# deevinandu/Distributed-Multi-Agent-SLAM-Swarm-Robotics-System

Hardware: NVIDIA B200
Metric: beam_cell_updates_per_sec (higher is better)
Workload: dtype f64+u32

## Files before the change

### distributed-multi-agent-slam-swarm-robotics-system_b200/csrc/beam_expand.cuh

```cuda
#pragma once
#include "sincos_dd.cuh"

namespace occ {

struct Geom {
    double ox, oy, res;
    double inv_res;
    int size_x, size_y;
    int win_x0, win_y0, win_w, win_h;
};

struct Beam {
    int x0, y0, x1, y1;
    int hit;
    int valid;
    int slow;
};

#define OCC_MAX_DIST_M 1.20
#define OCC_MIN_DIST_M 0.05
#define OCC_CELL_LIMIT 1073741824.0

OCC_HD float load_f32_unaligned(const uint8_t* p) {
    uint32_t v = (uint32_t)p[0] | ((uint32_t)p[1] << 8) | ((uint32_t)p[2] << 16) | ((uint32_t)p[3] << 24);
#if defined(__CUDA_ARCH__)
    return __uint_as_float(v);
#else
    float f;
    __builtin_memcpy(&f, &v, 4);
    return f;
#endif
}

OCC_HD double cell_quotient(double w, double o, double res) { return OCC_DDIV(OCC_DADD(w, -o), res); }

OCC_HD bool quotient_in_range(double q) { return fabs(q) < OCC_CELL_LIMIT; }

OCC_HD int trunc_cell(double q) {
#if defined(__CUDA_ARCH__)
    return __double2int_rz(q);
#else
    return (int)q;
#endif
}

OCC_HD double screening_tolerance(double r, double o, double yaw, double inv_res) {
    return OCC_DMUL(OCC_DMUL(fabs(r) + fabs(o) + fabs(yaw) + 11.0, inv_res), 0x1p-47);
}

OCC_HD bool near_cell_boundary(double q, double tol) { return !(fabs(q - rint(q)) > tol); }

struct LibSinCos {
    OCC_HD_MEMBER void operator()(double a, double* s, double* c) const {
#if defined(__CUDA_ARCH__)
        sincos(a, s, c);
#else
        *s = sin(a);
        *c = cos(a);
#endif
    }
};

OCC_HD double sensor_angle(int s) {
    const double h = 0x1.921fb54442d18p+0;
    return s == 0 ? 0.0 : (s == 1 ? h : (s == 2 ? 0x1.921fb54442d18p+1 : -h));
}

template <class FastSinCos>
OCC_HD void expand_beam(const Geom& g, double rx, double ry, double ryaw, int x0, int y0, bool origin_ok,
                        int sensor, float dist_f32, double sn, double cs, double tolx, double toly,
                        const FastSinCos& fsc, Beam* b) {
    double dist = (double)dist_f32;
    bool hit = (OCC_MIN_DIST_M < dist) && (dist <= OCC_MAX_DIST_M);
    double range = hit ? dist : OCC_MAX_DIST_M;
    double qx = OCC_DMUL(OCC_DADD(OCC_DADD(rx, OCC_DMUL(range, cs)), -g.ox), g.inv_res);
    double qy = OCC_DMUL(OCC_DADD(OCC_DADD(ry, OCC_DMUL(range, sn)), -g.oy), g.inv_res);
    int slow = 0;
    if (near_cell_boundary(qx, tolx) || near_cell_boundary(qy, toly)) {
        double ang = OCC_DADD(ryaw, sensor_angle(sensor));
        double s2, c2;
        if (!sincos_dd(ang, &s2, &c2)) fsc(ang, &s2, &c2);
        qx = cell_quotient(OCC_DADD(rx, OCC_DMUL(range, c2)), g.ox, g.res);
        qy = cell_quotient(OCC_DADD(ry, OCC_DMUL(range, s2)), g.oy, g.res);
        slow = 1;
    }
    b->hit = hit ? 1 : 0;
    b->slow = slow;
    b->x0 = x0;
    b->y0 = y0;
    bool ok = origin_ok && quotient_in_range(qx) && quotient_in_range(qy);
    b->valid = ok ? 1 : 0;
    b->x1 = ok ? trunc_cell(qx) : 0;
    b->y1 = ok ? trunc_cell(qy) : 0;
}

enum { PKT_OK = 0, PKT_DROPPED = 1, PKT_BAD_POSE = 2 };

OCC_HD int decode_packet(const uint8_t* p, long long k, const int32_t* agent_idx, const double* drift,
                         const double* agent_off, int n_agents,
                         double* rx, double* ry, double* ryaw, float dist[4], int* agent_out = nullptr) {
    if (!(p[0] == 'Q' && p[1] == 'S' && p[2] == 'R' && p[3] == 'L')) return PKT_DROPPED;
    long long agent = agent_idx ? (long long)agent_idx[k] : (long long)p[4];
    if (agent < 1 || agent > n_agents) return PKT_DROPPED;
// ... 107 lines not shown
```

### distributed-multi-agent-slam-swarm-robotics-system_b200/csrc/occgrid_tiled.cu

```cuda
#include "common.cuh"

namespace occ {

constexpr int kTT = 256;
constexpr int kChunkPk = 2048;
constexpr int kChunkMin = 256;
constexpr int kItemsPerCta = 3;
constexpr int kMaxWindowBytes = 100 * 1024;

struct TilePlanHeader {
    unsigned int n_items, n_active, total_records, work_counter, resolve_counter, overflow;
    unsigned int active_count;
    unsigned int pad;
};

__device__ __forceinline__ int home_tile(const Geom& g, const TileGeom& tg, double rx, double ry) {
    const double qx = cell_quotient(rx, g.ox, g.res), qy = cell_quotient(ry, g.oy, g.res);
    if (!quotient_in_range(qx) || !quotient_in_range(qy)) return -1;
    const int px = trunc_cell(qx) - g.win_x0 + tg.pad, py = trunc_cell(qy) - g.win_y0 + tg.pad;
    if (px < tg.pad - tg.reach || py < tg.pad - tg.reach || px >= tg.pad + g.win_w + tg.reach ||
        py >= tg.pad + g.win_h + tg.reach)
        return -1;
    return (py >> kTileShift) * tg.tiles_x + (px >> kTileShift);
}

constexpr int kPkPerCta = 2048;
constexpr int kSub = kPkPerCta / kTT;
constexpr int kHash = 4096;
constexpr unsigned int kEmpty = 0xffffffffu;
static_assert(kHash >= 2 * kPkPerCta, "hash table must stay at most half full");

__device__ __forceinline__ int hash_insert(unsigned int* keys, unsigned int tile) {
    unsigned int h = (tile * 2654435761u) >> 20;
    for (;;) {
        const unsigned int old = atomicCAS(&keys[h], kEmpty, tile);
        if (old == kEmpty || old == tile) return (int)h;
        h = (h + 1) & (kHash - 1);
    }
}

constexpr int kHashPerThread = kHash / kTT;

__device__ __forceinline__ void flush_tile_counts(const unsigned int* s_keys, const unsigned int* s_vals,
                                                  unsigned int* __restrict__ tile_count, unsigned int* __restrict__ active,
                                                  TilePlanHeader* __restrict__ hdr) {
    unsigned int key[kHashPerThread], old[kHashPerThread];
#pragma unroll
    for (int j = 0; j < kHashPerThread; ++j) {
        const int i = j * kTT + threadIdx.x;
        key[j] = s_keys[i];
        old[j] = 1u;
        if (key[j] != kEmpty) old[j] = atomicAdd(&tile_count[key[j]], s_vals[i]);
    }
#pragma unroll
    for (int j = 0; j < kHashPerThread; ++j)
        if (key[j] != kEmpty && old[j] == 0u) active[atomicAdd(&hdr->active_count, 1u)] = key[j];
}

__device__ __forceinline__ void reserve_tile_ranges(const unsigned int* s_keys, unsigned int* s_vals,
                                                    const unsigned int* __restrict__ tile_offset, unsigned int* __restrict__ tile_cursor) {
    unsigned int key[kHashPerThread], base[kHashPerThread], off[kHashPerThread];
#pragma unroll
    for (int j = 0; j < kHashPerThread; ++j) {
        const int i = j * kTT + threadIdx.x;
        key[j] = s_keys[i];
        base[j] = off[j] = 0u;
        if (key[j] != kEmpty) { off[j] = tile_offset[key[j]]; base[j] = atomicAdd(&tile_cursor[key[j]], s_vals[i]); }
    }
#pragma unroll
    for (int j = 0; j < kHashPerThread; ++j)
        if (key[j] != kEmpty) s_vals[j * kTT + threadIdx.x] = off[j] + base[j];
}

constexpr size_t kBinSmem = (size_t)kTT * kMaxRecStride + 2 * kHash * sizeof(unsigned int) + kPkPerCta * sizeof(unsigned short);
constexpr unsigned int kNoSlot = 0xffffu;

template <bool kMaps = false>
__global__ void __launch_bounds__(kTT)
k_home_bin(Geom g, TileGeom tg, const uint8_t* __restrict__ pkts, long long n, int stride,
           const int32_t* __restrict__ agent_idx, const double* __restrict__ drift,
           const double* __restrict__ agent_off, int n_agents,
           unsigned int* __restrict__ tile_count, PoseRec* __restrict__ recs, unsigned int* __restrict__ local_bins, uint2* __restrict__ runs,
           unsigned int* __restrict__ seg_count, unsigned int* __restrict__ active, TilePlanHeader* __restrict__ hdr,
           uint64_t* counters) {
    extern __shared__ __align__(16) uint8_t s_bin[];
    uint8_t* const s_rec = s_bin;
    unsigned int* const s_keys = reinterpret_cast<unsigned int*>(s_bin + kTT * kMaxRecStride);
    unsigned int* const s_vals = s_keys + kHash;
    unsigned short* const s_slot = reinterpret_cast<unsigned short*>(s_vals + kHash);
    __shared__ unsigned int s_wsum[kTT / 32];
    for (int i = threadIdx.x; i < kHash; i += kTT) { s_keys[i] = kEmpty; s_vals[i] = 0u; }
    unsigned long long c[OCCGRID_C_HITS + 1] = {};
    const long long cta_first = (long long)blockIdx.x * kPkPerCta;
    constexpr int kVec = (kTT * kMaxRecStride / 16 + kTT - 1) / kTT;
    uint4 pre[kVec];
    auto prefetch = [&](int sub) {
        const long long first = cta_first + (long long)sub * kTT;
        const long long left = n - first;
        const size_t bytes = left <= 0 ? 0 : (size_t)min((long long)kTT, left) * stride;
        const uint4* s4 = reinterpret_cast<const uint4*>(pkts + (size_t)first * stride);
#pragma unroll
        for (int j = 0; j < kVec; ++j) {
            const size_t i = (size_t)j * kTT + threadIdx.x;
            pre[j] = (i * 16 + 16 <= bytes) ? __ldg(s4 + i) : make_uint4(0u, 0u, 0u, 0u);
        }
    };
    const bool vec_ok = (reinterpret_cast<uintptr_t>(pkts) & 15) == 0 && ((kTT * stride) & 15) == 0;
    if (vec_ok) prefetch(0);
    for (int sub = 0; sub < kSub; ++sub) {
        const long long first = cta_first + (long long)sub * kTT;
        if (first >= n) break;
        const int count = (int)min((long long)kTT, n - first);
        __syncthreads();
        if (vec_ok) {
            const size_t bytes = (size_t)count * stride;
            uint4* d4 = reinterpret_cast<uint4*>(s_rec);
#pragma unroll
            for (int j = 0; j < kVec; ++j) {
                const size_t i = (size_t)j * kTT + threadIdx.x;
                if (i * 16 + 16 <= bytes) d4[i] = pre[j];
            }
            for (size_t i = (bytes / 16) * 16 + threadIdx.x; i < bytes; i += kTT) s_rec[i] = __ldg(pkts + (size_t)first * stride + i);
            if (sub + 1 < kSub) prefetch(sub + 1);
        } else {
            stage_records(pkts + (size_t)first * stride, (size_t)count * stride, s_rec);
        }
        __syncthreads();
        if ((int)threadIdx.x < count) {
            const long long k = first + threadIdx.x;
            double rx, ry, ryaw;
            float dist[4];
            c[OCCGRID_C_PACKETS] += 1;
            unsigned int slot = kNoSlot;
            int agent = 1;
            const int st = decode_packet(s_rec + threadIdx.x * stride, k, agent_idx, drift, agent_off, n_agents, &rx, &ry, &ryaw, dist,
                                         kMaps ? &agent : nullptr);
            if (st == PKT_DROPPED) c[OCCGRID_C_DROPPED] += 1;
            else if (st == PKT_BAD_POSE) c[OCCGRID_C_BAD_POSE] += 1;
            else {
                c[OCCGRID_C_ACCEPTED] += 1;
                c[OCCGRID_C_BEAMS] += 4;
#pragma unroll
                for (int s = 0; s < 4; ++s) {
                    const double d = (double)dist[s];
                    c[OCCGRID_C_HITS] += (OCC_MIN_DIST_M < d && d <= OCC_MAX_DIST_M) ? 1 : 0;
                }
                int tile = home_tile(g, tg, rx, ry);
                if (kMaps && tile >= 0) tile += (agent - 1) * tg.n_tiles;
                if (tile >= 0) {
                    slot = (unsigned int)hash_insert(s_keys, (unsigned int)tile);
                    atomicAdd(&s_vals[slot], 1u);
                    PoseRec r;
                    r.rx = rx; r.ry = ry; r.yaw = (float)ryaw;
                    r.d[0] = dist[0]; r.d[1] = dist[1]; r.d[2] = dist[2]; r.d[3] = dist[3];
                    r.k = (unsigned int)k;
                    r.tile = tile; r.pad = 0;
                    recs[k] = r;
                }
            }
            s_slot[sub * kTT + threadIdx.x] = (unsigned short)slot;
        }
    }
    __syncthreads();
    unsigned int key[kHashPerThread], rank[kHashPerThread];
#pragma unroll
    for (int j = 0; j < kHashPerThread; ++j) {
        const int i = j * kTT + threadIdx.x;
        key[j] = s_keys[i];
        rank[j] = 0u;
        if (key[j] != kEmpty) rank[j] = atomicAdd(&tile_count[key[j]], s_vals[i]);
    }
    const int lane = threadIdx.x & 31, warp = threadIdx.x >> 5;
    unsigned int mine = 0u;
#pragma unroll
    for (int j = 0; j < kHashPerThread; ++j) mine += key[j] != kEmpty ? s_vals[j * kTT + threadIdx.x] + 0x10000u : 0u;
    unsigned int inc = mine;
#pragma unroll
    for (int o = 1; o < 32; o <<= 1) { const unsigned int u = __shfl_up_sync(0xffffffffu, inc, o); if (lane >= o) inc += u; }
    if (lane == 31) s_wsum[warp] = inc;
    __syncthreads();
    unsigned int pos = inc - mine, n_local = 0u;
#pragma unroll
    for (int w = 0; w < kTT / 32; ++w) {
        pos += w < warp ? s_wsum[w] : 0u;
        n_local += s_wsum[w];
    }
    n_local &= 0xffffu;
    if (threadIdx.x == 0) seg_count[blockIdx.x] = n_local;
    const size_t seg0 = (size_t)blockIdx.x * kPkPerCta;
#pragma unroll
    for (int j = 0; j < kHashPerThread; ++j) {
        if (key[j] == kEmpty) continue;
        const int i = j * kTT + threadIdx.x;
        const unsigned int run = pos >> 16, begin = pos & 0xffffu;
        runs[seg0 + run] = make_uint2(key[j], rank[j] - begin);
        pos += s_vals[i] + 0x10000u;
        s_keys[i] = run;
        s_vals[i] = begin;
        if (rank[j] == 0u) active[atomicAdd(&hdr->active_count, 1u)] = key[j];
    }
    __syncthreads();
    unsigned int* const s_local = reinterpret_cast<unsigned int*>(s_rec);
    const int n_seg = (int)min((long long)kPkPerCta, n - (long long)seg0);
    for (int j = threadIdx.x; j < n_seg; j += kTT) {
        const unsigned int slot = s_slot[j];
        if (slot != kNoSlot) s_local[atomicAdd(&s_vals[slot], 1u)] = (s_keys[slot] << 16) | (unsigned int)j;
    }
    __syncthreads();
    for (unsigned int j = threadIdx.x; j < n_local; j += kTT) local_bins[seg0 + j] = s_local[j];
    __syncthreads();
    block_add_counters(c, reinterpret_cast<unsigned long long*>(s_rec), counters);
}

__global__ void __launch_bounds__(kTT)
k_place_runs(const unsigned int* __restrict__ local_bins, const uint2* __restrict__ runs, const unsigned int* __restrict__ seg_count,
             const unsigned int* __restrict__ tile_offset, const TilePlanHeader* __restrict__ hdr, unsigned int* __restrict__ bins) {
    if (hdr->overflow) return;
    const size_t seg0 = (size_t)blockIdx.x * kPkPerCta;
    const int n_local = (int)seg_count[blockIdx.x];
    unsigned int e[kSub], off[kSub];
    uint2 d[kSub];
#pragma unroll
    for (int sub = 0; sub < kSub; ++sub) {
        const int j = sub * kTT + threadIdx.x;
        e[sub] = j < n_local ? local_bins[seg0 + j] : kEmpty;
    }
#pragma unroll
    for (int sub = 0; sub < kSub; ++sub) d[sub] = e[sub] != kEmpty ? runs[seg0 + (e[sub] >> 16)] : make_uint2(0u, 0u);
#pragma unroll
    for (int sub = 0; sub < kSub; ++sub) off[sub] = e[sub] != kEmpty ? tile_offset[d[sub].x] : 0u;
#pragma unroll
    for (int sub = 0; sub < kSub; ++sub)
        if (e[sub] != kEmpty) bins[off[sub] + d[sub].y + (unsigned int)(sub * kTT + threadIdx.x)] = (unsigned int)(seg0 + (e[sub] & 0xffffu));
}

__device__ __forceinline__ int chunk_valid(const SegInfo& seg, long long chunk, long long* addr0) {
    const long long a0 = chunk * kSegChunk;
    *addr0 = a0;
    const unsigned int sg = (unsigned int)(a0 / seg.seg_cap);
    const unsigned int j0 = (unsigned int)(a0 - (long long)sg * seg.seg_cap);
    unsigned int cnt = seg.d_counts ? seg.d_counts[sg] : seg.host_count;
    if (cnt > seg.seg_cap) cnt = seg.seg_cap;
    return cnt > j0 ? (int)min((unsigned int)kSegChunk, cnt - j0) : 0;
}

__global__ void __launch_bounds__(kTT)
k_home_count_poses(Geom g, TileGeom tg, const PoseRec* __restrict__ recs, const int* __restrict__ in_tiles, SegInfo seg, long long n_chunks,
                   int tiles_in_records,
                   unsigned int* __restrict__ tile_count, int* __restrict__ tile_ids,
                   unsigned int* __restrict__ active, TilePlanHeader* __restrict__ hdr, uint64_t* counters) {
    __shared__ unsigned int s_keys[kHash];
    __shared__ unsigned int s_vals[kHash];
    __shared__ unsigned long long s_acc[(OCCGRID_C_HITS + 1) * 32];
    unsigned long long c[OCCGRID_C_HITS + 1] = {};
    for (long long chunk = blockIdx.x; chunk < n_chunks; chunk += gridDim.x) {
        long long addr0;
        const int valid = chunk_valid(seg, chunk, &addr0);
        if (valid == 0) continue;
        for (int i = threadIdx.x; i < kHash; i += kTT) { s_keys[i] = kEmpty; s_vals[i] = 0u; }
        __syncthreads();
        if (tiles_in_records) {
            int tl[kSub];
#pragma unroll
            for (int sub = 0; sub < kSub; ++sub) {
// ... 268 lines not shown
    else      asm volatile("red.shared.max.u32 [%0], %1;" ::"r"(addr), "r"(v) : "memory");
}

template <bool kAdd>
__device__ __forceinline__ void walk_beam_masked(unsigned int win, int pitch, int x, int y, int ddx, int ddy,
                                                 unsigned int v_free, bool hit, bool skip_first, const unsigned int* s_mask) {
    const int dx = abs(ddx), dy = abs(ddy);
    const bool xmajor = dx >= dy;
    const int dmaj = xmajor ? dx : dy, dmin = xmajor ? dy : dx;
    const int sx4 = ddx > 0 ? 4 : -4;
    const int sy4 = (ddy > 0 ? pitch : -pitch) * 4;
    const int step_maj = xmajor ? sx4 : sy4, step_min = xmajor ? sy4 : sx4;
    unsigned int mask = s_mask[dmaj * (dmaj + 1) / 2 + dmin];
    unsigned int a = win + (unsigned int)(y * pitch + x) * 4u;
    const unsigned int a_end = a + (unsigned int)((ddy * pitch + ddx) * 4);
    int rem = dmaj;
    if (rem > 0) {
        if (!skip_first) smem_red<kAdd>(a, v_free);
        a += step_maj + ((mask & 1u) ? step_min : 0);
        mask >>= 1;
        --rem;
    }
    while (rem >= 8) {
#pragma unroll
        for (int j = 0; j < 8; ++j) {
            smem_red<kAdd>(a, v_free);
            a += step_maj + ((mask & (1u << j)) ? step_min : 0);
        }
        mask >>= 8;
        rem -= 8;
    }
    if (rem >= 4) {
#pragma unroll
        for (int j = 0; j < 4; ++j) {
            smem_red<kAdd>(a, v_free);
            a += step_maj + ((mask & (1u << j)) ? step_min : 0);
        }
        mask >>= 4;
        rem -= 4;
    }
    for (; rem > 0; --rem) {
        smem_red<kAdd>(a, v_free);
        a += step_maj + ((mask & 1u) ? step_min : 0);
        mask >>= 1;
    }
    if (hit && !(dmaj == 0 && skip_first && !kAdd)) smem_red<kAdd>(a_end, kAdd ? 0x10000u : (v_free | 1u));
}

struct RouteSmem {
    unsigned int cnt[kMaxBands];
    unsigned int off[kMaxBands + 1];
    unsigned int base[kMaxBands];
};

__device__ __forceinline__ unsigned int lds_u32_at(const unsigned int* __restrict__ words, unsigned int byte_off) {
    const unsigned int w = byte_off >> 2, sh = (byte_off & 3u) * 8u;
    return __funnelshift_r(words[w], words[w + 1], sh);
}

__device__ __forceinline__ int decode_packet_smem(const unsigned int* __restrict__ words, unsigned int byte_off, long long k,
                                                  const int32_t* agent_idx, const double* drift, const double* agent_off,
                                                  int n_agents, double* rx, double* ry, float* yaw, float dist[4]) {
    if (lds_u32_at(words, byte_off) != 0x4c525351u) return PKT_DROPPED;
    const unsigned int b4 = lds_u32_at(words, byte_off + 4);
    const long long agent = agent_idx ? (long long)agent_idx[k] : (long long)(b4 & 0xffu);
    if (agent < 1 || agent > n_agents) return PKT_DROPPED;
    const unsigned int b8 = lds_u32_at(words, byte_off + 8), b12 = lds_u32_at(words, byte_off + 12),
                       b16 = lds_u32_at(words, byte_off + 16);
    double x = (double)__uint_as_float(__funnelshift_r(b4, b8, 8));
    double y = (double)__uint_as_float(__funnelshift_r(b8, b12, 8));
    const float fyaw = __uint_as_float(__funnelshift_r(b12, b16, 8));
    x = OCC_DADD(x, agent_off[2 * agent + 0]);
    y = OCC_DADD(y, agent_off[2 * agent + 1]);
    if (drift) {
        const double2 dv = *reinterpret_cast<const double2*>(drift + 2 * k);
        x = OCC_DADD(x, dv.x);
        y = OCC_DADD(y, dv.y);
    }
    if (!(isfinite(x) && isfinite(y) && isfinite(fyaw))) return PKT_BAD_POSE;
    *rx = x; *ry = y; *yaw = fyaw;
    const unsigned int c24 = lds_u32_at(words, byte_off + 24), c28 = lds_u32_at(words, byte_off + 28),
                       c32 = lds_u32_at(words, byte_off + 32), c36 = lds_u32_at(words, byte_off + 36),
                       c40 = lds_u32_at(words, byte_off + 40);
    dist[0] = __uint_as_float(__funnelshift_r(c24, c28, 8));
    dist[1] = __uint_as_float(__funnelshift_r(c28, c32, 8));
    dist[2] = __uint_as_float(__funnelshift_r(c32, c36, 8));
    dist[3] = __uint_as_float(__funnelshift_r(c36, c40, 8));
    return PKT_OK;
}

__device__ __forceinline__ bool robot_cell(double r, double o, double res, double inv_res, int* cell) {
    double q = OCC_DMUL(OCC_DADD(r, -o), inv_res);
    const double tol = OCC_DMUL(OCC_DMUL(fabs(r) + fabs(o) + 11.0, inv_res), 0x1p-47);
    if (near_cell_boundary(q, tol)) q = cell_quotient(r, o, res);
    if (!quotient_in_range(q)) return false;
    *cell = trunc_cell(q);
    return true;
}

struct RouteStats { unsigned int a, b; };

constexpr int kRouteSubs = kRouteSubsPerItem;
constexpr int kRoutePerThread = kRouteItemPk / kTT;
static_assert(kRouteItemPk % kTT == 0 && kRoutePerThread >= 1 && kRoutePerThread <= 4, "route sub-batch = 1..4 packets per thread");

struct RoutePk {
    double rx, ry;
    float yaw, d[4];
    int band0, nb, tile0, tile1;
    unsigned int rank0, rank1;
};

__device__ __forceinline__ void route_decode(const RouteJob& J, const unsigned int* s_buf, int slot, long long k, RoutePk& P,
                                             RouteStats& st_acc) {
    P.band0 = -1; P.nb = 0; P.tile0 = P.tile1 = -1; P.rank0 = P.rank1 = 0u;
    const int st = decode_packet_smem(s_buf, (unsigned int)slot * (unsigned int)J.stride, k, J.agent_idx, J.drift, J.agent_off,
                                      J.n_agents, &P.rx, &P.ry, &P.yaw, P.d);
    st_acc.a += 1u + (st == PKT_OK ? 0x10000u : 0u);
    st_acc.b += st == PKT_DROPPED ? 1u : 0u;
    if (st != PKT_OK) return;
    unsigned int hits = 0;
#pragma unroll
    for (int s2 = 0; s2 < 4; ++s2) {
        const double dd = (double)P.d[s2];
        hits += (OCC_MIN_DIST_M < dd && dd <= OCC_MAX_DIST_M) ? 1u : 0u;
    }
    st_acc.b += hits << 16;
    int gx, gy;
    if (!(robot_cell(P.rx, J.ox, J.res, J.inv_res, &gx) && robot_cell(P.ry, J.oy, J.res, J.inv_res, &gy))) return;
    const int reach = J.reach;
    if (gx < -reach || gx >= J.size_x + reach) return;
    const int tcol = (gx + J.pad) >> kTileShift;
    for (int b = 0; b < J.n_bands; ++b) {
        if (gy - reach < J.band_y0[b + 1]) {
            const int py = gy - J.band_y0[b];
            if (py >= -reach) {
                P.band0 = b; P.nb = 1;
                P.tile0 = ((py + J.pad) >> kTileShift) * J.tiles_x + tcol;
                if (b + 1 < J.n_bands && gy + reach >= J.band_y0[b + 1]) {
                    P.nb = 2;
                    P.tile1 = ((gy - J.band_y0[b + 1] + J.pad) >> kTileShift) * J.tiles_x + tcol;
                }
            }
            break;
        }
    }
}

__device__ __forceinline__ void route_rank(RouteSmem& S, RoutePk& P, int lane, unsigned int lt) {
    const unsigned int p0 = __match_any_sync(0xffffffffu, P.band0);
    if (P.band0 >= 0) {
// ... 208 lines not shown
        if (threadIdx.x == 0) next_pos = atomicAdd(&hdr->work_counter, 1u);
        __syncthreads();
        {
            const int lx_lo = max(0, g.win_x0 - wx0), lx_hi = min(side, g.win_x0 + g.win_w - wx0);
            const int ly_lo = max(0, g.win_y0 - wy0), ly_hi = min(side, g.win_y0 + g.win_h - wy0);
            const int lane = threadIdx.x & 31, warp = threadIdx.x >> 5;
            for (int ly = warp; ly < side; ly += kTT / 32) {
                unsigned int* row = s_win + ly * pitch;
                const bool row_in = ly >= ly_lo && ly < ly_hi;
                unsigned int* out = plane + (size_t)(wy0 + ly - g.win_y0) * g.win_w + (wx0 - g.win_x0);
                for (int lx = lane; lx < side; lx += 32) {
                    const unsigned int v = row[lx];
                    if (!v) continue;
                    if (!kRoute) row[lx] = 0u;
                    if (!(row_in && lx >= lx_lo && lx < lx_hi)) continue;
                    if (kCounts)
                        atomicAdd(reinterpret_cast<unsigned long long*>(plane) + ((size_t)(wy0 + ly - g.win_y0) * g.win_w + (wx0 - g.win_x0) + lx),
                                  ((unsigned long long)(v >> 16) << 32) | (unsigned long long)(v & 0xffffu));
                    else
                        atomicMax(out + lx, v);
                }
            }
        }
        if (threadIdx.x == 0) s_next[turn ^ 1] = next_pos;
        __syncthreads();
    }
    if (kRoute && job.counters) {
        __syncthreads();
        const unsigned long long pk = rs.a & 0xffffu, acc = rs.a >> 16, drp = rs.b & 0xffffu, hits = rs.b >> 16;
        const unsigned long long rc[6] = {pk, acc, drp, pk - acc - drp, 4ull * acc, hits};
        block_add_counters(rc, s_acc, job.counters);
    }
    if (counters) {
        __syncthreads();
        const int lane = threadIdx.x & 31, warp = threadIdx.x >> 5;
#pragma unroll
        for (int i = 0; i < 3; ++i) {
            unsigned long long x = c[i];
#pragma unroll
            for (int o = 16; o > 0; o >>= 1) x += __shfl_xor_sync(0xffffffffu, x, o);
            if (lane == 0) s_acc[i * 32 + warp] = x;
        }
        __syncthreads();
        if (threadIdx.x < 3) {
            unsigned long long t = 0;
            for (int w = 0; w < kTT / 32; ++w) t += s_acc[threadIdx.x * 32 + w];
            const int slot = threadIdx.x == 0 ? OCCGRID_C_UPDATES : (threadIdx.x == 1 ? OCCGRID_C_SLOWPATH : OCCGRID_C_OWNED_UPDATES);
            if (t) atomicAdd(reinterpret_cast<unsigned long long*>(counters) + slot, t);
        }
    }
}

constexpr int kResolveSplit = 8;

template <bool kMaps = false>
__global__ void __launch_bounds__(kTT)
k_home_resolve(Geom g, TileGeom tg, const unsigned int* __restrict__ active, TilePlanHeader* __restrict__ hdr,
               unsigned int* __restrict__ stamps, int8_t* __restrict__ grid) {
    __shared__ unsigned int s_item;
    const unsigned int n_work = hdr->n_active * kResolveSplit;
    const int side = tg.win_side;
    const int lane = threadIdx.x & 31, warp = threadIdx.x >> 5;
    for (;;) {
        __syncthreads();
        if (threadIdx.x == 0) s_item = atomicAdd(&hdr->resolve_counter, 1u);
        __syncthreads();
        const unsigned int it = s_item;
        if (it >= n_work) break;
        const unsigned int key = active[it / kResolveSplit];
        const unsigned int map = kMaps ? key / (unsigned int)tg.n_tiles : 0u;
        const unsigned int t = key - map * (unsigned int)tg.n_tiles;
        const size_t map_off = kMaps ? (size_t)map * ((size_t)g.win_w * g.win_h) : 0;
        unsigned int* __restrict__ const plane = stamps + map_off;
        int8_t* __restrict__ const map_grid = grid + map_off;
        const int part = (int)(it % kResolveSplit);
        const int ttx = t % tg.tiles_x, tty = t / tg.tiles_x;
        const int wx0 = -tg.pad + (ttx << kTileShift) - tg.reach;
        const int wy0 = -tg.pad + (tty << kTileShift) - tg.reach;
        const int lx_lo = max(0, -wx0), lx_hi = min(side, g.win_w - wx0);
        const int ly_lo = max(0, -wy0), ly_hi = min(side, g.win_h - wy0);
        if (lx_hi <= lx_lo) continue;
        for (int ly = ly_lo + part * (kTT / 32) + warp; ly < ly_hi; ly += kResolveSplit * (kTT / 32)) {
            const size_t row = (size_t)(wy0 + ly) * g.win_w + wx0;
            for (int lx = lx_lo + lane; lx < lx_hi; lx += 32) {
                const unsigned int s = plane[row + lx];
                if (s) {
                    map_grid[row + lx] = (s & 1u) ? OCCGRID_CELL_OCCUPIED : OCCGRID_CELL_FREE;
                    plane[row + lx] = 0u;
                }
            }
        }
    }
}


static int g_raycast_cta_cap = 0;
void set_raycast_cta_cap(int cap) { g_raycast_cta_cap = cap < 0 ? 0 : cap; }

struct TiledLayout {
    size_t off_stamps, off_count, off_offset, off_cursor, off_active, off_hdr, off_items, off_ids, off_bins, off_local, off_runs,
        off_segs, off_recs, total;
    unsigned long long max_records;
    unsigned int max_items;
};

static TiledLayout tiled_layout(const occgrid_geom* geom, int64_t max_records, bool packets, int n_maps = 1) {
    TiledLayout L;
    const TileGeom tg = tile_geom(geom);
    const size_t n_keys = (size_t)n_maps * tg.n_tiles;
    L.max_records = (unsigned long long)max_records;
    unsigned long long items = L.max_records / kChunkMin + (unsigned long long)n_keys + 1;
    if (items > L.max_records + 1) items = L.max_records + 1;
    L.max_items = (unsigned int)items;
    size_t o = 0;
    L.off_stamps = o; o += align_up((size_t)geom->win_w * geom->win_h * 4 * (size_t)n_maps, 256);
    L.off_count = o;  o += align_up((n_keys + 1) * 4, 256);
    L.off_offset = o; o += align_up((n_keys + 1) * 4, 256);
    L.off_cursor = o; o += align_up((n_keys + 1) * 4, 256);
    L.off_active = o; o += align_up((n_keys + 1) * 4, 256);
    L.off_hdr = o;    o += 256;
    L.off_items = o;  o += align_up((size_t)L.max_items * sizeof(uint4), 256);
    L.off_ids = o;    o += packets ? 0 : align_up((size_t)L.max_records * sizeof(int), 256);
    L.off_bins = o;   o += align_up((size_t)L.max_records * sizeof(unsigned int), 256);
    L.off_local = o;  o += packets ? align_up((size_t)L.max_records * sizeof(unsigned int), 256) : 0;
    L.off_runs = o;   o += packets ? align_up((size_t)L.max_records * sizeof(uint2), 256) : 0;
    L.off_segs = o;   o += packets ? align_up((size_t)(L.max_records + kPkPerCta - 1) / kPkPerCta * sizeof(unsigned int), 256) : 0;
    L.off_recs = o;   o += packets ? align_up((size_t)L.max_records * sizeof(PoseRec), 256) : 0;
    L.total = o;
    return L;
}

bool tiled_supported(const occgrid_geom* geom, int n_maps) {
    const TileGeom tg = tile_geom(geom);
    return (size_t)tg.win_side * tg.pitch * 4 <= (size_t)kMaxWindowBytes && (long long)n_maps * tg.n_tiles <= (1ll << 24);
}

size_t tiled_workspace_bytes(const occgrid_geom* geom, int n_maps, int64_t max_packets) {
    return tiled_layout(geom, max_packets < 1 ? 1 : max_packets, true, n_maps).total;
}

size_t tiled_band_workspace_bytes(const occgrid_geom* geom, int n_segs, int64_t seg_cap) {
// ... 39 lines not shown

template <bool kCounts, bool kRoute, bool kMaps = false>
static int launch_raycast(const Geom& g, const TileGeom& tg, const TiledPtrs& P, const PoseRec* recs, int ordinals_in_records,
                          unsigned int* plane, uint64_t* d_counters, int have_items, const RouteJob& job, cudaStream_t st) {
    const size_t smem = raycast_smem(tg, kRoute);
    static thread_local size_t configured = 0;
    if (smem > configured) {
        OCC_CUDA_TRY(cudaFuncSetAttribute(k_home_raycast<kCounts, kRoute, kMaps>, cudaFuncAttributeMaxDynamicSharedMemorySize, (int)smem));
        configured = smem;
    }
    int ctas_per_sm = 1;
    if (cudaOccupancyMaxActiveBlocksPerMultiprocessor(&ctas_per_sm, k_home_raycast<kCounts, kRoute, kMaps>, kTT, smem) != cudaSuccess || ctas_per_sm < 1)
        ctas_per_sm = 1;
    if (g_raycast_cta_cap > 0 && ctas_per_sm > g_raycast_cta_cap) ctas_per_sm = g_raycast_cta_cap;
    ProfileScope ps(K_TILE_RAYCAST, st);
    k_home_raycast<kCounts, kRoute, kMaps><<<device_sm_count() * ctas_per_sm, kTT, smem, st>>>(g, tg, P.items, P.hdr, P.bins, recs,
                                                                                               ordinals_in_records, plane, d_counters,
                                                                                               have_items, job);
    return OCCGRID_OK;
}

static unsigned int plan_target_items() { return (unsigned int)device_sm_count() * 3u * (unsigned int)kItemsPerCta; }

static int grid_chunks(long long n_chunks) {
    long long b = n_chunks < 1 ? 1 : n_chunks;
    const long long cap = (long long)device_sm_count() * 8;
    return (int)(b < cap ? b : cap);
}

int integrate_tiled(const occgrid_geom* geom, const PacketBatch& batch, const PoseRec* d_poses, int ordinals_in_records, Output kind,
                    void* d_out, void* d_ws, size_t ws_bytes, uint64_t* d_counters, cudaStream_t st) {
    const int64_t n = batch.n;
    const bool maps = kind == Output::kAgentMaps;
    const TiledLayout L = tiled_layout(geom, n, d_poses == nullptr, maps ? batch.n_agents : 1);
    if (ws_bytes < L.total) {
        set_last_error("workspace %zu B < %zu B needed by TILED for %lld records", ws_bytes, L.total, (long long)n);
        return OCCGRID_E_WORKSPACE;
    }
    const TiledPtrs P = tiled_ptrs(L, d_ws);
    const PoseRec* recs = d_poses ? d_poses : P.recs;
    const Geom g = to_geom(geom);
    const TileGeom tg = tile_geom(geom);
    const unsigned int blocks = (unsigned int)((n + kPkPerCta - 1) / kPkPerCta);
    SegInfo seg;
    seg.n_segs = 1; seg.seg_cap = (unsigned int)align_up((size_t)n, kSegChunk); seg.d_counts = nullptr; seg.host_count = (unsigned int)n;
    const long long n_chunks = (n + kSegChunk - 1) / kSegChunk;
    {
        ProfileScope ps(K_TILE_COUNT, st);
        if (d_poses) {
            k_home_count_poses<<<grid_chunks(n_chunks), kTT, 0, st>>>(g, tg, d_poses, nullptr, seg, n_chunks, 0, P.tile_count, P.tile_ids, P.active,
                                                                      P.hdr, d_counters);
        } else {
            const auto bin = maps ? k_home_bin<true> : k_home_bin<false>;
            OCC_CUDA_TRY(cudaFuncSetAttribute(bin, cudaFuncAttributeMaxDynamicSharedMemorySize, (int)kBinSmem));
            bin<<<blocks, kTT, kBinSmem, st>>>(g, tg, batch.pkts, n, batch.stride, batch.agent_idx, batch.drift, batch.agent_off, batch.n_agents,
                                               P.tile_count, P.recs, P.local_bins, P.runs, P.seg_count, P.active, P.hdr, d_counters);
        }
    }
    {
        ProfileScope ps(K_TILE_SCAN, st);
        k_tile_plan<<<1, 1024, 0, st>>>(P.tile_count, P.tile_offset, P.tile_cursor, P.items, L.max_items, P.active, L.max_records, P.hdr,
                                        d_counters, plan_target_items());
    }
    {
        ProfileScope ps(K_TILE_SCATTER, st);
        if (d_poses) k_home_scatter_segs<<<grid_chunks(n_chunks), kTT, 0, st>>>(seg, n_chunks, P.tile_ids, P.tile_offset, P.tile_cursor, P.hdr, P.bins);
        else         k_place_runs<<<blocks, kTT, 0, st>>>(P.local_bins, P.runs, P.seg_count, P.tile_offset, P.hdr, P.bins);
    }
    RouteJob none = {};
    unsigned int* const plane = kind == Output::kCounts ? reinterpret_cast<unsigned int*>(d_out) : P.stamps;
    if (kind == Output::kCounts) launch_raycast<true, false>(g, tg, P, recs, ordinals_in_records, plane, d_counters, 1, none, st);
    else if (maps)               launch_raycast<false, false, true>(g, tg, P, recs, ordinals_in_records, plane, d_counters, 1, none, st);
    else                         launch_raycast<false, false>(g, tg, P, recs, ordinals_in_records, plane, d_counters, 1, none, st);
    if (kind != Output::kCounts) {
        ProfileScope ps(K_TILE_RESOLVE, st);
        const auto resolve = maps ? k_home_resolve<true> : k_home_resolve<false>;
        resolve<<<device_sm_count() * 8, kTT, 0, st>>>(g, tg, P.active, P.hdr, P.stamps, reinterpret_cast<int8_t*>(d_out));
    }
    OCC_CUDA_TRY(cudaGetLastError());
    return OCCGRID_OK;
}

int tiled_prepare_poses(const occgrid_geom* geom, const PoseRec* d_recs, const int* d_tiles, const SegInfo& seg, int tiles_in_records,
                        void* d_ws, size_t ws_bytes, uint64_t* d_counters, cudaStream_t st) {
    const int64_t max_records = (int64_t)seg.n_segs * seg.seg_cap;
    const TiledLayout L = tiled_layout(geom, max_records, false);
    if (ws_bytes < L.total) {
        set_last_error("workspace %zu B < %zu B needed by the band step for %lld record addresses", ws_bytes, L.total, (long long)max_records);
        return OCCGRID_E_WORKSPACE;
    }
    const TiledPtrs P = tiled_ptrs(L, d_ws);
    const Geom g = to_geom(geom);
    const TileGeom tg = tile_geom(geom);
    const long long n_chunks = max_records / kSegChunk;
    {
        ProfileScope ps(K_TILE_COUNT, st);
        k_home_count_poses<<<grid_chunks(n_chunks), kTT, 0, st>>>(g, tg, d_recs, d_tiles, seg, n_chunks, tiles_in_records, P.tile_count, P.tile_ids,
                                                                  P.active, P.hdr, d_counters);
    }
    {
        ProfileScope ps(K_TILE_SCAN, st);
        k_tile_plan<<<1, 1024, 0, st>>>(P.tile_count, P.tile_offset, P.tile_cursor, P.items, L.max_items, P.active, L.max_records, P.hdr,
                                        d_counters, plan_target_items());
    }
    {
        ProfileScope ps(K_TILE_SCATTER, st);
        k_home_scatter_segs<<<grid_chunks(n_chunks), kTT, 0, st>>>(seg, n_chunks, P.tile_ids, P.tile_offset, P.tile_cursor, P.hdr, P.bins);
    }
// ... 32 lines not shown
```

Baseline: 676.4 billion.

## Make home binning persistent with a cp.async multi-stage packet pipeline

Converts k_home_bin into a persistent kernel sized to resident CTAs that loops over segments and stages packet records into shared memory through a three-slot cp.async pipeline, so loads for upcoming chunks overlap decoding of the current one. Packets are decoded from shared memory with funnel shifts, the home cell is computed with a screened fast quotient instead of always dividing, and counters are kept as 32-bit locals. The resolve kernel drops its atomic work queue for a grid-stride loop and processes two rows and four words per lane to raise memory-level parallelism. The cost is more shared memory per CTA, reuse of a staging slot for the local bin list, and more complex synchronisation.

After: 695.4 billion, median of 6. +2.8%, better.

```diff
diff --git a/distributed-multi-agent-slam-swarm-robotics-system_b200/csrc/beam_expand.cuh b/distributed-multi-agent-slam-swarm-robotics-system_b200/csrc/beam_expand.cuh
--- a/distributed-multi-agent-slam-swarm-robotics-system_b200/csrc/beam_expand.cuh
+++ b/distributed-multi-agent-slam-swarm-robotics-system_b200/csrc/beam_expand.cuh
@@ -49,6 +49,15 @@
 }
 
 OCC_HD bool near_cell_boundary(double q, double tol) { return !(fabs(q - rint(q)) > tol); }
+
+OCC_HD bool robot_cell(double r, double o, double res, double inv_res, int* cell) {
+    double q = OCC_DMUL(OCC_DADD(r, -o), inv_res);
+    const double tol = OCC_DMUL(OCC_DMUL(fabs(r) + fabs(o) + 11.0, inv_res), 0x1p-47);
+    if (near_cell_boundary(q, tol)) q = cell_quotient(r, o, res);
+    if (!quotient_in_range(q)) return false;
+    *cell = trunc_cell(q);
+    return true;
+}
 
 struct LibSinCos {
     OCC_HD_MEMBER void operator()(double a, double* s, double* c) const {
diff --git a/distributed-multi-agent-slam-swarm-robotics-system_b200/csrc/occgrid_tiled.cu b/distributed-multi-agent-slam-swarm-robotics-system_b200/csrc/occgrid_tiled.cu
--- a/distributed-multi-agent-slam-swarm-robotics-system_b200/csrc/occgrid_tiled.cu
+++ b/distributed-multi-agent-slam-swarm-robotics-system_b200/csrc/occgrid_tiled.cu
@@ -14,14 +14,56 @@
     unsigned int pad;
 };
 
-__device__ __forceinline__ int home_tile(const Geom& g, const TileGeom& tg, double rx, double ry) {
-    const double qx = cell_quotient(rx, g.ox, g.res), qy = cell_quotient(ry, g.oy, g.res);
-    if (!quotient_in_range(qx) || !quotient_in_range(qy)) return -1;
-    const int px = trunc_cell(qx) - g.win_x0 + tg.pad, py = trunc_cell(qy) - g.win_y0 + tg.pad;
+__device__ __forceinline__ int home_tile_of_cell(const Geom& g, const TileGeom& tg, int cx, int cy) {
+    const int px = cx - g.win_x0 + tg.pad, py = cy - g.win_y0 + tg.pad;
     if (px < tg.pad - tg.reach || py < tg.pad - tg.reach || px >= tg.pad + g.win_w + tg.reach ||
         py >= tg.pad + g.win_h + tg.reach)
         return -1;
     return (py >> kTileShift) * tg.tiles_x + (px >> kTileShift);
+}
+
+__device__ __forceinline__ int home_tile(const Geom& g, const TileGeom& tg, double rx, double ry) {
+    const double qx = cell_quotient(rx, g.ox, g.res), qy = cell_quotient(ry, g.oy, g.res);
+    if (!quotient_in_range(qx) || !quotient_in_range(qy)) return -1;
+    return home_tile_of_cell(g, tg, trunc_cell(qx), trunc_cell(qy));
+}
+
+__device__ __forceinline__ unsigned int lds_u32_at(const unsigned int* __restrict__ words, unsigned int byte_off) {
+    const unsigned int w = byte_off >> 2, sh = (byte_off & 3u) * 8u;
+    return __funnelshift_r(words[w], words[w + 1], sh);
+}
+
+__device__ __forceinline__ int decode_packet_smem(const unsigned int* __restrict__ words, unsigned int byte_off, long long k,
+                                                  const int32_t* agent_idx, const double* drift, const double* agent_off,
+                                                  int n_agents, double* rx, double* ry, float* yaw, float dist[4],
+                                                  int* agent_out = nullptr) {
+    if (lds_u32_at(words, byte_off) != 0x4c525351u) return PKT_DROPPED;
+    const unsigned int b4 = lds_u32_at(words, byte_off + 4);
+    const long long agent = agent_idx ? (long long)agent_idx[k] : (long long)(b4 & 0xffu);
+    if (agent < 1 || agent > n_agents) return PKT_DROPPED;
+    if (agent_out) *agent_out = (int)agent;
+    const unsigned int b8 = lds_u32_at(words, byte_off + 8), b12 = lds_u32_at(words, byte_off + 12),
+                       b16 = lds_u32_at(words, byte_off + 16);
+    double x = (double)__uint_as_float(__funnelshift_r(b4, b8, 8));
+    double y = (double)__uint_as_float(__funnelshift_r(b8, b12, 8));
+    const float fyaw = __uint_as_float(__funnelshift_r(b12, b16, 8));
+    x = OCC_DADD(x, agent_off[2 * agent + 0]);
+    y = OCC_DADD(y, agent_off[2 * agent + 1]);
+    if (drift) {
+        const double2 dv = *reinterpret_cast<const double2*>(drift + 2 * k);
+        x = OCC_DADD(x, dv.x);
+        y = OCC_DADD(y, dv.y);
+    }
+    if (!(isfinite(x) && isfinite(y) && isfinite(fyaw))) return PKT_BAD_POSE;
+    *rx = x; *ry = y; *yaw = fyaw;
+    const unsigned int c24 = lds_u32_at(words, byte_off + 24), c28 = lds_u32_at(words, byte_off + 28),
+                       c32 = lds_u32_at(words, byte_off + 32), c36 = lds_u32_at(words, byte_off + 36),
+                       c40 = lds_u32_at(words, byte_off + 40);
+    dist[0] = __uint_as_float(__funnelshift_r(c24, c28, 8));
+    dist[1] = __uint_as_float(__funnelshift_r(c28, c32, 8));
+    dist[2] = __uint_as_float(__funnelshift_r(c32, c36, 8));
+    dist[3] = __uint_as_float(__funnelshift_r(c36, c40, 8));
+    return PKT_OK;
 }
 
 constexpr int kPkPerCta = 2048;
@@ -72,11 +114,24 @@
         if (key[j] != kEmpty) s_vals[j * kTT + threadIdx.x] = off[j] + base[j];
 }
 
-constexpr size_t kBinSmem = (size_t)kTT * kMaxRecStride + 2 * kHash * sizeof(unsigned int) + kPkPerCta * sizeof(unsigned short);
+constexpr int kStages = 3;
 constexpr unsigned int kNoSlot = 0xffffu;
+constexpr size_t kBinHashBytes = 2 * kHash * sizeof(unsigned int) + kPkPerCta * sizeof(unsigned short);
+static_assert(kPkPerCta * sizeof(unsigned int) <= (size_t)kTT * 41, "a segment's local bin list must fit one staging slot");
+
+__host__ __device__ __forceinline__ unsigned int bin_slot_bytes(int stride) { return ((unsigned int)(kTT * stride) + 8u + 15u) & ~15u; }
+static size_t bin_smem_bytes(int stride) { return (size_t)kStages * bin_slot_bytes(stride) + kBinHashBytes; }
+
+__device__ __forceinline__ void stage_async(const uint8_t* __restrict__ src, size_t bytes, uint8_t* dst) {
+    const unsigned int d0 = (unsigned int)__cvta_generic_to_shared(dst);
+    for (size_t i = threadIdx.x; i * 16 < bytes; i += kTT) {
+        const unsigned int n = (unsigned int)min((size_t)16, bytes - i * 16);
+        asm volatile("cp.async.cg.shared.global [%0], [%1], 16, %2;" ::"r"(d0 + (unsigned int)i * 16u), "l"(src + i * 16), "r"(n) : "memory");
+    }
+}
 
 template <bool kMaps = false>
-__global__ void __launch_bounds__(kTT)
+__global__ void __launch_bounds__(kTT, 3)
 k_home_bin(Geom g, TileGeom tg, const uint8_t* __restrict__ pkts, long long n, int stride,
            const int32_t* __restrict__ agent_idx, const double* __restrict__ drift,
            const double* __restrict__ agent_off, int n_agents,
@@ -84,74 +139,75 @@
            unsigned int* __restrict__ seg_count, unsigned int* __restrict__ active, TilePlanHeader* __restrict__ hdr,
            uint64_t* counters) {
     extern __shared__ __align__(16) uint8_t s_bin[];
-    uint8_t* const s_rec = s_bin;
-    unsigned int* const s_keys = reinterpret_cast<unsigned int*>(s_bin + kTT * kMaxRecStride);
+    const unsigned int slot_bytes = bin_slot_bytes(stride);
+    uint8_t* const s_stage = s_bin;
+    unsigned int* const s_keys = reinterpret_cast<unsigned int*>(s_bin + kStages * slot_bytes);
     unsigned int* const s_vals = s_keys + kHash;
     unsigned short* const s_slot = reinterpret_cast<unsigned short*>(s_vals + kHash);
     __shared__ unsigned int s_wsum[kTT / 32];
     for (int i = threadIdx.x; i < kHash; i += kTT) { s_keys[i] = kEmpty; s_vals[i] = 0u; }
-    unsigned long long c[OCCGRID_C_HITS + 1] = {};
-    const long long cta_first = (long long)blockIdx.x * kPkPerCta;
-    constexpr int kVec = (kTT * kMaxRecStride / 16 + kTT - 1) / kTT;
-    uint4 pre[kVec];
-    auto prefetch = [&](int sub) {
-        const long long first = cta_first + (long long)sub * kTT;
-        const long long left = n - first;
-        const size_t bytes = left <= 0 ? 0 : (size_t)min((long long)kTT, left) * stride;
-        const uint4* s4 = reinterpret_cast<const uint4*>(pkts + (size_t)first * stride);
-#pragma unroll
-        for (int j = 0; j < kVec; ++j) {
-            const size_t i = (size_t)j * kTT + threadIdx.x;
-            pre[j] = (i * 16 + 16 <= bytes) ? __ldg(s4 + i) : make_uint4(0u, 0u, 0u, 0u);
-        }
+    unsigned int n_pk = 0u, n_drop = 0u, n_bad = 0u, n_hits = 0u;
+    const long long n_segs = (n + kPkPerCta - 1) / kPkPerCta;
+    const bool async = (reinterpret_cast<uintptr_t>(pkts) & 15) == 0;
+    long long p_seg = blockIdx.x;
+    int p_sub = 0, p_slot = 0;
+    auto stage_next = [&]() {
+        if (p_seg < n_segs) {
+            const long long first = p_seg * kPkPerCta + (long long)p_sub * kTT;
+            const size_t bytes = (size_t)min((long long)kTT, n - first) * stride;
+            uint8_t* const dst = s_stage + p_slot * slot_bytes;
+            if (async) stage_async(pkts + (size_t)first * stride, bytes, dst);
+            else       stage_records(pkts + (size_t)first * stride, bytes, dst);
+            if ((long long)(p_sub + 1) * kTT < min((long long)kPkPerCta, n - p_seg * kPkPerCta)) ++p_sub;
+            else { p_seg += gridDim.x; p_sub = 0; }
+            p_slot = p_slot + 1 == kStages ? 0 : p_slot + 1;
+        }
+        if (async) asm volatile("cp.async.commit_group;" ::: "memory");
     };
-    const bool vec_ok = (reinterpret_cast<uintptr_t>(pkts) & 15) == 0 && ((kTT * stride) & 15) == 0;
-    if (vec_ok) prefetch(0);
-    for (int sub = 0; sub < kSub; ++sub) {
-        const long long first = cta_first + (long long)sub * kTT;
-        if (first >= n) break;
-        const int count = (int)min((long long)kTT, n - first);
-        __syncthreads();
-        if (vec_ok) {
-            const size_t bytes = (size_t)count * stride;
-            uint4* d4 = reinterpret_cast<uint4*>(s_rec);
-#pragma unroll
-            for (int j = 0; j < kVec; ++j) {
-                const size_t i = (size_t)j * kTT + threadIdx.x;
-                if (i * 16 + 16 <= bytes) d4[i] = pre[j];
-            }
-            for (size_t i = (bytes / 16) * 16 + threadIdx.x; i < bytes; i += kTT) s_rec[i] = __ldg(pkts + (size_t)first * stride + i);
-            if (sub + 1 < kSub) prefetch(sub + 1);
-        } else {
-            stage_records(pkts + (size_t)first * stride, (size_t)count * stride, s_rec);
-        }
-        __syncthreads();
-        if ((int)threadIdx.x < count) {
-            const long long k = first + threadIdx.x;
-            double rx, ry, ryaw;
-            float dist[4];
-            c[OCCGRID_C_PACKETS] += 1;
+#pragma unroll
+    for (int i = 0; i < kStages - 1; ++i) stage_next();
+    int buf = 0;
+    for (long long seg = blockIdx.x; seg < n_segs; seg += gridDim.x) {
+        const long long seg0 = seg * kPkPerCta;
+        const int n_seg = (int)min((long long)kPkPerCta, n - seg0);
+        for (int sub = 0; sub * kTT < n_seg; ++sub, buf = buf + 1 == kStages ? 0 : buf + 1) {
+            const long long k = seg0 + sub * kTT + threadIdx.x;
+            const bool mine = sub * kTT + (int)threadIdx.x < n_seg;
+            double2 dv = make_double2(0.0, 0.0);
+            if (drift && mine) dv = make_double2(drift[2 * k], drift[2 * k + 1]);
+            asm volatile("cp.async.wait_group %0;" ::"n"(kStages - 2) : "memory");
+            __syncthreads();
+            stage_next();
+            if (!mine) continue;
+            double rx, ry;
+            float yaw, dist[4];
+            int agent = 1;
             unsigned int slot = kNoSlot;
-            int agent = 1;
-            const int st = decode_packet(s_rec + threadIdx.x * stride, k, agent_idx, drift, agent_off, n_agents, &rx, &ry, &ryaw, dist,
-                                         kMaps ? &agent : nullptr);
-            if (st == PKT_DROPPED) c[OCCGRID_C_DROPPED] += 1;
-            else if (st == PKT_BAD_POSE) c[OCCGRID_C_BAD_POSE] += 1;
+            n_pk += 1u;
+            int st = decode_packet_smem(reinterpret_cast<const unsigned int*>(s_stage + buf * slot_bytes), threadIdx.x * (unsigned int)stride,
+                                        k, agent_idx, nullptr, agent_off, n_agents, &rx, &ry, &yaw, dist, &agent);
+            if (st == PKT_OK && drift) {
+                rx = OCC_DADD(rx, dv.x);
+                ry = OCC_DADD(ry, dv.y);
+                if (!(isfinite(rx) && isfinite(ry))) st = PKT_BAD_POSE;
+            }
+            if (st == PKT_DROPPED) n_drop += 1u;
+            else if (st == PKT_BAD_POSE) n_bad += 1u;
             else {
-                c[OCCGRID_C_ACCEPTED] += 1;
-                c[OCCGRID_C_BEAMS] += 4;
 #pragma unroll
                 for (int s = 0; s < 4; ++s) {
                     const double d = (double)dist[s];
-                    c[OCCGRID_C_HITS] += (OCC_MIN_DIST_M < d && d <= OCC_MAX_DIST_M) ? 1 : 0;
+                    n_hits += (OCC_MIN_DIST_M < d && d <= OCC_MAX_DIST_M) ? 1u : 0u;
                 }
-                int tile = home_tile(g, tg, rx, ry);
+                int cx, cy, tile = -1;
+                if (robot_cell(rx, g.ox, g.res, g.inv_res, &cx) && robot_cell(ry, g.oy, g.res, g.inv_res, &cy))
+                    tile = home_tile_of_cell(g, tg, cx, cy);
                 if (kMaps && tile >= 0) tile += (agent - 1) * tg.n_tiles;
                 if (tile >= 0) {
                     slot = (unsigned int)hash_insert(s_keys, (unsigned int)tile);
                     atomicAdd(&s_vals[slot], 1u);
                     PoseRec r;
-                    r.rx = rx; r.ry = ry; r.yaw = (float)ryaw;
+                    r.rx = rx; r.ry = ry; r.yaw = yaw;
                     r.d[0] = dist[0]; r.d[1] = dist[1]; r.d[2] = dist[2]; r.d[3] = dist[3];
                     r.k = (unsigned int)k;
                     r.tile = tile; r.pad = 0;
@@ -160,56 +216,58 @@
             }
             s_slot[sub * kTT + threadIdx.x] = (unsigned short)slot;
         }
-    }
+        __syncthreads();
+        unsigned int key[kHashPerThread], rank[kHashPerThread];
+#pragma unroll
+        for (int j = 0; j < kHashPerThread; ++j) {
+            const int i = j * kTT + threadIdx.x;
+            key[j] = s_keys[i];
+            rank[j] = 0u;
+            if (key[j] != kEmpty) rank[j] = atomicAdd(&tile_count[key[j]], s_vals[i]);
+        }
+        const int lane = threadIdx.x & 31, warp = threadIdx.x >> 5;
+        unsigned int mine = 0u;
+#pragma unroll
+        for (int j = 0; j < kHashPerThread; ++j) mine += key[j] != kEmpty ? s_vals[j * kTT + threadIdx.x] + 0x10000u : 0u;
+        unsigned int inc = mine;
+#pragma unroll
+        for (int o = 1; o < 32; o <<= 1) { const unsigned int u = __shfl_up_sync(0xffffffffu, inc, o); if (lane >= o) inc += u; }
+        if (lane == 31) s_wsum[warp] = inc;
+        __syncthreads();
+        unsigned int pos = inc - mine, n_local = 0u;
+#pragma unroll
+        for (int w = 0; w < kTT / 32; ++w) {
+            pos += w < warp ? s_wsum[w] : 0u;
+            n_local += s_wsum[w];
+        }
+        n_local &= 0xffffu;
+        if (threadIdx.x == 0) seg_count[seg] = n_local;
+#pragma unroll
+        for (int j = 0; j < kHashPerThread; ++j) {
+            if (key[j] == kEmpty) continue;
+            const int i = j * kTT + threadIdx.x;
+            const unsigned int run = pos >> 16, begin = pos & 0xffffu;
+            runs[seg0 + run] = make_uint2(key[j], rank[j] - begin);
+            pos += s_vals[i] + 0x10000u;
+            s_keys[i] = run;
+            s_vals[i] = begin;
+            if (rank[j] == 0u) active[atomicAdd(&hdr->active_count, 1u)] = key[j];
+        }
+        __syncthreads();
+        unsigned int* const s_local = reinterpret_cast<unsigned int*>(s_stage + (buf == 0 ? kStages - 1 : buf - 1) * slot_bytes);
+        for (int j = threadIdx.x; j < n_seg; j += kTT) {
+            const unsigned int slot = s_slot[j];
+            if (slot != kNoSlot) s_local[atomicAdd(&s_vals[slot], 1u)] = (s_keys[slot] << 16) | (unsigned int)j;
+        }
+        __syncthreads();
+        for (unsigned int j = threadIdx.x; j < n_local; j += kTT) local_bins[seg0 + j] = s_local[j];
+        for (int i = threadIdx.x; i < kHash; i += kTT) { s_keys[i] = kEmpty; s_vals[i] = 0u; }
+    }
+    asm volatile("cp.async.wait_all;" ::: "memory");
     __syncthreads();
-    unsigned int key[kHashPerThread], rank[kHashPerThread];
-#pragma unroll
-    for (int j = 0; j < kHashPerThread; ++j) {
-        const int i = j * kTT + threadIdx.x;
-        key[j] = s_keys[i];
-        rank[j] = 0u;
-        if (key[j] != kEmpty) rank[j] = atomicAdd(&tile_count[key[j]], s_vals[i]);
-    }
-    const int lane = threadIdx.x & 31, warp = threadIdx.x >> 5;
-    unsigned int mine = 0u;
-#pragma unroll
-    for (int j = 0; j < kHashPerThread; ++j) mine += key[j] != kEmpty ? s_vals[j * kTT + threadIdx.x] + 0x10000u : 0u;
-    unsigned int inc = mine;
-#pragma unroll
-    for (int o = 1; o < 32; o <<= 1) { const unsigned int u = __shfl_up_sync(0xffffffffu, inc, o); if (lane >= o) inc += u; }
-    if (lane == 31) s_wsum[warp] = inc;
-    __syncthreads();
-    unsigned int pos = inc - mine, n_local = 0u;
-#pragma unroll
-    for (int w = 0; w < kTT / 32; ++w) {
-        pos += w < warp ? s_wsum[w] : 0u;
-        n_local += s_wsum[w];
-    }
-    n_local &= 0xffffu;
-    if (threadIdx.x == 0) seg_count[blockIdx.x] = n_local;
-    const size_t seg0 = (size_t)blockIdx.x * kPkPerCta;
-#pragma unroll
-    for (int j = 0; j < kHashPerThread; ++j) {
-        if (key[j] == kEmpty) continue;
-        const int i = j * kTT + threadIdx.x;
-        const unsigned int run = pos >> 16, begin = pos & 0xffffu;
-        runs[seg0 + run] = make_uint2(key[j], rank[j] - begin);
-        pos += s_vals[i] + 0x10000u;
-        s_keys[i] = run;
-        s_vals[i] = begin;
-        if (rank[j] == 0u) active[atomicAdd(&hdr->active_count, 1u)] = key[j];
-    }
-    __syncthreads();
-    unsigned int* const s_local = reinterpret_cast<unsigned int*>(s_rec);
-    const int n_seg = (int)min((long long)kPkPerCta, n - (long long)seg0);
-    for (int j = threadIdx.x; j < n_seg; j += kTT) {
-        const unsigned int slot = s_slot[j];
-        if (slot != kNoSlot) s_local[atomicAdd(&s_vals[slot], 1u)] = (s_keys[slot] << 16) | (unsigned int)j;
-    }
-    __syncthreads();
-    for (unsigned int j = threadIdx.x; j < n_local; j += kTT) local_bins[seg0 + j] = s_local[j];
-    __syncthreads();
-    block_add_counters(c, reinterpret_cast<unsigned long long*>(s_rec), counters);
+    const unsigned int n_acc = n_pk - n_drop - n_bad;
+    const unsigned long long c[OCCGRID_C_HITS + 1] = {n_pk, n_acc, n_drop, n_bad, 4ull * n_acc, n_hits};
+    block_add_counters(c, reinterpret_cast<unsigned long long*>(s_stage), counters);
 }
 
 __global__ void __launch_bounds__(kTT)
@@ -584,51 +642,6 @@
     unsigned int off[kMaxBands + 1];
     unsigned int base[kMaxBands];
 };
-
-__device__ __forceinline__ unsigned int lds_u32_at(const unsigned int* __restrict__ words, unsigned int byte_off) {
-    const unsigned int w = byte_off >> 2, sh = (byte_off & 3u) * 8u;
-    return __funnelshift_r(words[w], words[w + 1], sh);
-}
-
-__device__ __forceinline__ int decode_packet_smem(const unsigned int* __restrict__ words, unsigned int byte_off, long long k,
-                                                  const int32_t* agent_idx, const double* drift, const double* agent_off,
-                                                  int n_agents, double* rx, double* ry, float* yaw, float dist[4]) {
-    if (lds_u32_at(words, byte_off) != 0x4c525351u) return PKT_DROPPED;
-    const unsigned int b4 = lds_u32_at(words, byte_off + 4);
-    const long long agent = agent_idx ? (long long)agent_idx[k] : (long long)(b4 & 0xffu);
-    if (agent < 1 || agent > n_agents) return PKT_DROPPED;
-    const unsigned int b8 = lds_u32_at(words, byte_off + 8), b12 = lds_u32_at(words, byte_off + 12),
-                       b16 = lds_u32_at(words, byte_off + 16);
-    double x = (double)__uint_as_float(__funnelshift_r(b4, b8, 8));
-    double y = (double)__uint_as_float(__funnelshift_r(b8, b12, 8));
-    const float fyaw = __uint_as_float(__funnelshift_r(b12, b16, 8));
-    x = OCC_DADD(x, agent_off[2 * agent + 0]);
-    y = OCC_DADD(y, agent_off[2 * agent + 1]);
-    if (drift) {
-        const double2 dv = *reinterpret_cast<const double2*>(drift + 2 * k);
-        x = OCC_DADD(x, dv.x);
-        y = OCC_DADD(y, dv.y);
-    }
-    if (!(isfinite(x) && isfinite(y) && isfinite(fyaw))) return PKT_BAD_POSE;
-    *rx = x; *ry = y; *yaw = fyaw;
-    const unsigned int c24 = lds_u32_at(words, byte_off + 24), c28 = lds_u32_at(words, byte_off + 28),
-                       c32 = lds_u32_at(words, byte_off + 32), c36 = lds_u32_at(words, byte_off + 36),
-                       c40 = lds_u32_at(words, byte_off + 40);
-    dist[0] = __uint_as_float(__funnelshift_r(c24, c28, 8));
-    dist[1] = __uint_as_float(__funnelshift_r(c28, c32, 8));
-    dist[2] = __uint_as_float(__funnelshift_r(c32, c36, 8));
-    dist[3] = __uint_as_float(__funnelshift_r(c36, c40, 8));
-    return PKT_OK;
-}
-
-__device__ __forceinline__ bool robot_cell(double r, double o, double res, double inv_res, int* cell) {
-    double q = OCC_DMUL(OCC_DADD(r, -o), inv_res);
-    const double tol = OCC_DMUL(OCC_DMUL(fabs(r) + fabs(o) + 11.0, inv_res), 0x1p-47);
-    if (near_cell_boundary(q, tol)) q = cell_quotient(r, o, res);
-    if (!quotient_in_range(q)) return false;
-    *cell = trunc_cell(q);
-    return true;
-}
 
 struct RouteStats { unsigned int a, b; };
 
@@ -943,21 +956,16 @@
 }
 
 constexpr int kResolveSplit = 8;
+constexpr int kResolveWords = 4;
 
 template <bool kMaps = false>
 __global__ void __launch_bounds__(kTT)
 k_home_resolve(Geom g, TileGeom tg, const unsigned int* __restrict__ active, TilePlanHeader* __restrict__ hdr,
                unsigned int* __restrict__ stamps, int8_t* __restrict__ grid) {
-    __shared__ unsigned int s_item;
     const unsigned int n_work = hdr->n_active * kResolveSplit;
     const int side = tg.win_side;
     const int lane = threadIdx.x & 31, warp = threadIdx.x >> 5;
-    for (;;) {
-        __syncthreads();
-        if (threadIdx.x == 0) s_item = atomicAdd(&hdr->resolve_counter, 1u);
-        __syncthreads();
-        const unsigned int it = s_item;
-        if (it >= n_work) break;
+    for (unsigned int it = blockIdx.x; it < n_work; it += gridDim.x) {
         const unsigned int key = active[it / kResolveSplit];
         const unsigned int map = kMaps ? key / (unsigned int)tg.n_tiles : 0u;
         const unsigned int t = key - map * (unsigned int)tg.n_tiles;
@@ -971,13 +979,23 @@
         const int lx_lo = max(0, -wx0), lx_hi = min(side, g.win_w - wx0);
         const int ly_lo = max(0, -wy0), ly_hi = min(side, g.win_h - wy0);
         if (lx_hi <= lx_lo) continue;
-        for (int ly = ly_lo + part * (kTT / 32) + warp; ly < ly_hi; ly += kResolveSplit * (kTT / 32)) {
-            const size_t row = (size_t)(wy0 + ly) * g.win_w + wx0;
-            for (int lx = lx_lo + lane; lx < lx_hi; lx += 32) {
-                const unsigned int s = plane[row + lx];
-                if (s) {
-                    map_grid[row + lx] = (s & 1u) ? OCCGRID_CELL_OCCUPIED : OCCGRID_CELL_FREE;
-                    plane[row + lx] = 0u;
+        constexpr int kRowStep = kResolveSplit * (kTT / 32);
+        for (int ly = ly_lo + part * (kTT / 32) + warp; ly < ly_hi; ly += 2 * kRowStep) {
+            const bool two = ly + kRowStep < ly_hi;
+            const size_t row0 = (size_t)(wy0 + ly) * g.win_w + wx0, row1 = row0 + (size_t)kRowStep * g.win_w;
+            for (int lx0 = lx_lo + lane; lx0 < lx_hi; lx0 += 32 * kResolveWords) {
+                unsigned int s0[kResolveWords], s1[kResolveWords];
+#pragma unroll
+                for (int j = 0; j < kResolveWords; ++j) {
+                    const int lx = lx0 + 32 * j;
+                    s0[j] = lx < lx_hi ? plane[row0 + lx] : 0u;
+                    s1[j] = two && lx < lx_hi ? plane[row1 + lx] : 0u;
+                }
+#pragma unroll
+                for (int j = 0; j < kResolveWords; ++j) {
+                    const int lx = lx0 + 32 * j;
+                    if (s0[j]) { map_grid[row0 + lx] = (s0[j] & 1u) ? OCCGRID_CELL_OCCUPIED : OCCGRID_CELL_FREE; plane[row0 + lx] = 0u; }
+                    if (s1[j]) { map_grid[row1 + lx] = (s1[j] & 1u) ? OCCGRID_CELL_OCCUPIED : OCCGRID_CELL_FREE; plane[row1 + lx] = 0u; }
                 }
             }
         }
@@ -1123,8 +1141,12 @@
                                                                       P.hdr, d_counters);
         } else {
             const auto bin = maps ? k_home_bin<true> : k_home_bin<false>;
-            OCC_CUDA_TRY(cudaFuncSetAttribute(bin, cudaFuncAttributeMaxDynamicSharedMemorySize, (int)kBinSmem));
-            bin<<<blocks, kTT, kBinSmem, st>>>(g, tg, batch.pkts, n, batch.stride, batch.agent_idx, batch.drift, batch.agent_off, batch.n_agents,
+            const size_t smem = bin_smem_bytes(batch.stride);
+            OCC_CUDA_TRY(cudaFuncSetAttribute(bin, cudaFuncAttributeMaxDynamicSharedMemorySize, (int)smem));
+            int ctas_per_sm = 1;
+            if (cudaOccupancyMaxActiveBlocksPerMultiprocessor(&ctas_per_sm, bin, kTT, smem) != cudaSuccess || ctas_per_sm < 1) ctas_per_sm = 1;
+            const unsigned int resident = (unsigned int)(device_sm_count() * ctas_per_sm);
+            bin<<<blocks < resident ? blocks : resident, kTT, smem, st>>>(g, tg, batch.pkts, n, batch.stride, batch.agent_idx, batch.drift, batch.agent_off, batch.n_agents,
                                                P.tile_count, P.recs, P.local_bins, P.runs, P.seg_count, P.active, P.hdr, d_counters);
         }
     }
```
